# Hawkeye-FineGrained/Hawkeye

Measured on AMD Instinct MI355X. Metric: images/sec (train fwd+bwd) BCNN VGG-16 448^2 bs64, higher is better.
Workload: dtype f32; 1 GPU; BCNN_S2: VGG-16 448x448, per-GPU batch 64, 200 classes, SGD momentum 0.9, CE label_smoothing 0.1, full train step; global_batch=64, parallelism=dp1, memory_format=channels_last

## Files before the change

hawkeye_amd/csrc/api.hip:

```cpp
#include <cstdlib>
#include <cstring>

#include "hk_bgemm.h"
#include "../../include/hawkeye_hip.h"

namespace hk {

namespace {
struct Knob {
    const char* name;
    const char* env;
    int Tuning::*field;
};
const Knob kKnobs[] = {
    {"bcnn_generic", "HK_BCNN_GENERIC", &Tuning::bcnn_generic}, {"cbp_bin", "HK_CBP_BIN", &Tuning::cbp_bin},
    {"roi_bwd", "HK_ROI_BWD", &Tuning::roi_bwd},                {"linear_slabs", "HK_LINEAR_SLABS", &Tuning::linear_slabs},
    {"ns_tn", "HK_NS_TN", &Tuning::ns_tn},                      {"bwd_v", "HK_BWD_V", &Tuning::bwd_v},
    {"ns_streams", "HK_NS_STREAMS", &Tuning::ns_streams},        {"sched_b", "HK_SCHED_B", &Tuning::sched_b},
    {"ns_sym", "HK_NS_SYM", &Tuning::ns_sym},
    {"lin_walk", "HK_LIN_WALK", &Tuning::lin_walk},           {"bwd_fold", "HK_BWD_FOLD", &Tuning::bwd_fold},
    {"fwd_fold", "HK_FWD_FOLD", &Tuning::fwd_fold},             {"conv_wrw", "HK_CONV_WRW", &Tuning::conv_wrw},
    {"wrw_wgs", "HK_WRW_WGS", &Tuning::wrw_wgs},                {"peer_form", "HK_PEER_FORM", &Tuning::peer_form},
    {"wrw_split", "HK_WRW_SPLIT", &Tuning::wrw_split},          {"wrw_wide", "HK_WRW_WIDE", &Tuning::wrw_wide},
    {"conv_fwd", "HK_CONV_FWD", &Tuning::conv_fwd},             {"conv_bwd_data", "HK_CONV_BWD_DATA", &Tuning::conv_bwd_data},
    {"conv_epi", "HK_CONV_EPI", &Tuning::conv_epi},             {"conv_mfma", "HK_CONV_MFMA", &Tuning::conv_mfma},
};
Tuning from_env() {
    Tuning t;
    for (const Knob& k : kKnobs)
        if (const char* e = getenv(k.env)) t.*(k.field) = atoi(e);
    return t;
}
}

Tuning& tuning() {
    static Tuning t = from_env();
    return t;
}

}

using namespace hk;

extern "C" int hk_tuning_set(const char* name, int value) {
    if (!name) return HK_ERR_BAD_ARG;
    for (const Knob& k : kKnobs)
        if (!strcmp(name, k.name)) {
            tuning().*(k.field) = value;
            return HK_OK;
        }
    return HK_ERR_BAD_ARG;
}

extern "C" int hk_tuning_get(const char* name, int* value) {
    if (!name || !value) return HK_ERR_BAD_ARG;
    for (const Knob& k : kKnobs)
        if (!strcmp(name, k.name)) {
            *value = tuning().*(k.field);
            return HK_OK;
        }
    return HK_ERR_BAD_ARG;
}

extern "C" const char* hk_version(void) { return "hawkeye_hip 0.1 gfx950"; }

extern "C" int hk_bgemm_f32(const float* a, int lda, long long stride_a, int trans_a, const float* b, int ldb,
                            long long stride_b, int trans_b, float* c, int ldc, long long stride_c, int M, int N,
                            int K, int batch, float alpha, float beta, float diag, hk_stream_t stream) {
    if (!a || !b || !c) return HK_ERR_BAD_ARG;
    hipStream_t st = (hipStream_t)stream;
    const LdPlain la = trans_a ? make_plain(a, stride_a, lda, K, M) : make_plain(a, stride_a, lda, M, K);
    const LdPlain lb = trans_b ? make_plain(b, stride_b, ldb, N, K) : make_plain(b, stride_b, ldb, K, N);
    const EpAffine ep = make_affine(c, stride_c, ldc, alpha, nullptr, beta, diag);
    if (!trans_a && !trans_b) return bgemm_launch<true, false>(la, lb, ep, M, N, K, batch, st);
    if (!trans_a && trans_b) return bgemm_launch<true, true>(la, lb, ep, M, N, K, batch, st);
    if (trans_a && !trans_b) return bgemm_launch<false, false>(la, lb, ep, M, N, K, batch, st);
    return bgemm_launch<false, true>(la, lb, ep, M, N, K, batch, st);
}
```

hawkeye_amd/csrc/conv_wrw.hip:

```cpp
#include "hk_common.h"
#include "hk_partial_sum.h"
#include "hk_split_bf16.h"
#include "../../include/hawkeye_hip.h"

namespace hk {

constexpr int WRW_CI = 64;
constexpr int WRW_OT = 64;
constexpr int WRW_SW = 32;
constexpr int WRW_XROW = (WRW_SW + 2) * WRW_CI;
constexpr int WRW_DYROW = WRW_SW * WRW_OT;
constexpr int WRW_XF4 = WRW_XROW / 4;
constexpr int WRW_LDS = 4 * WRW_XROW + 2 * WRW_DYROW;
constexpr int WRW_MIN_ROWS = 4;
constexpr int WRW_MAX_WG = 512;

struct WrwStage {
    long long xoff[3], doff[2];
    bool xok[3], dok[2];
};

__device__ __forceinline__ bool wrw_load_x(const float* __restrict__ xi, const WrwStage& st, int r, int H, int W, int cin, f32x4 (&v)[3]) {
    const bool rok = r >= 0 && r < H;
    const float* row = xi + (long long)(r < 0 ? 0 : (r < H ? r : H - 1)) * W * cin;
#pragma unroll
    for (int u = 0; u < 3; ++u) HK_LOAD16_ASYNC(v[u], row + st.xoff[u]);
    return rok;
}
__device__ __forceinline__ void wrw_load_dy(const float* __restrict__ dyi, const WrwStage& st, int h, int H, int W, int Cout, f32x4 (&v)[2]) {
    const float* row = dyi + (long long)(h < H ? h : H - 1) * W * Cout;
#pragma unroll
    for (int u = 0; u < 2; ++u) HK_LOAD16_ASYNC(v[u], row + st.doff[u]);
}
__device__ __forceinline__ void wrw_loads_landed(f32x4 (&vx)[3], f32x4 (&vd)[2]) {
    __builtin_amdgcn_s_waitcnt(HK_VMCNT_IMM(0));
#pragma unroll
    for (int u = 0; u < 3; ++u) HK_PIN_LOADED(vx[u]);
#pragma unroll
    for (int u = 0; u < 2; ++u) HK_PIN_LOADED(vd[u]);
}
__device__ __forceinline__ void wrw_store_x(float* __restrict__ xs, int slot, const WrwStage& st, bool rok, const f32x4 (&v)[3]) {
    const f32x4 zero = {0.f, 0.f, 0.f, 0.f};
    f32x4* d = reinterpret_cast<f32x4*>(xs + slot * WRW_XROW) + threadIdx.x;
    d[0] = (rok && st.xok[0]) ? v[0] : zero;
    d[256] = (rok && st.xok[1]) ? v[1] : zero;
    if (threadIdx.x + 512 < WRW_XF4) d[512] = (rok && st.xok[2]) ? v[2] : zero;
}
__device__ __forceinline__ void wrw_store_dy(float* __restrict__ ds, int buf, const WrwStage& st, const f32x4 (&v)[2]) {
    const f32x4 zero = {0.f, 0.f, 0.f, 0.f};
    f32x4* d = reinterpret_cast<f32x4*>(ds + buf * WRW_DYROW) + threadIdx.x;
    d[0] = st.dok[0] ? v[0] : zero;
    d[256] = st.dok[1] ? v[1] : zero;
}

__global__ __launch_bounds__(256, 2) void conv3x3_wrw_kernel(const float* __restrict__ dy, const float* __restrict__ x,
                                                          float* __restrict__ part, int H, int W, int Cout, int nstrips, int nrb,
                                                          int rpb, int njobs) {
    __shared__ __attribute__((aligned(16))) float lds[WRW_LDS];
    float* xs = lds;
    float* ds = lds + 4 * WRW_XROW;
    const int tid = threadIdx.x, lane = tid & 63, l31 = lane & 31, hf = lane >> 5;
    const int wave = __builtin_amdgcn_readfirstlane(tid >> 6);
    const int oh = wave >> 1, ch = wave & 1;
    const int slice = blockIdx.y;
    const int jb = (int)((long long)blockIdx.x * njobs / gridDim.x), je = (int)((long long)(blockIdx.x + 1) * njobs / gridDim.x);

    f32x16 acc[9];
#pragma unroll
    for (int t = 0; t < 9; ++t)
#pragma unroll
        for (int i = 0; i < 16; ++i) acc[t][i] = 0.f;

    const int aoff = hf * WRW_OT + oh * 32 + l31;
    const int boff = hf * WRW_CI + ch * 32 + l31;

    for (int j = jb; j < je; ++j) {
        const int strip = j % nstrips, jr = j / nstrips;
        const int rb = jr % nrb;
        const long long n = jr / nrb;
        const int c0 = strip * WRW_SW, r0 = rb * rpb;
        const int nrows = (r0 + rpb < H ? r0 + rpb : H) - r0;
        const float* xi = x + n * H * W * WRW_CI;
        const float* dyi = dy + n * H * W * Cout + slice * WRW_OT;
        WrwStage st;
#pragma unroll
        for (int u = 0; u < 3; ++u) {
            const int idx = tid + 256 * u, col = c0 - 1 + (idx >> 4);
            st.xok[u] = idx < WRW_XF4 && col >= 0 && col < W;
            st.xoff[u] = (long long)(col < 0 ? 0 : (col < W ? col : W - 1)) * WRW_CI + 4 * (idx & 15);
        }
#pragma unroll
        for (int u = 0; u < 2; ++u) {
            const int idx = tid + 256 * u, col = c0 + (idx >> 4);
            st.dok[u] = col < W;
            st.doff[u] = (long long)(col < W ? col : W - 1) * Cout + 4 * (idx & 15);
        }
        f32x4 vx[3], vd[2];
        wrw_load_dy(dyi, st, r0, H, W, Cout, vd);
#pragma unroll
        for (int t = 0; t < 3; ++t) {
            const bool rok = wrw_load_x(xi, st, r0 - 1 + t, H, W, WRW_CI, vx);
            wrw_loads_landed(vx, vd);
            wrw_store_x(xs, t, st, rok, vx);
        }
        wrw_store_dy(ds, 0, st, vd);
        __syncthreads();
        for (int k = 0; k < nrows; ++k) {
            const bool rok = wrw_load_x(xi, st, r0 + k + 2, H, W, WRW_CI, vx);
            wrw_load_dy(dyi, st, r0 + k + 1, H, W, Cout, vd);
            const float* A = ds + (k & 1) * WRW_DYROW + aoff;
            const float* B0 = xs + (k & 3) * WRW_XROW + boff;
            const float* B1 = xs + ((k + 1) & 3) * WRW_XROW + boff;
            const float* B2 = xs + ((k + 2) & 3) * WRW_XROW + boff;
            float a = *HK_LDS_CONST(A), b[9];
#pragma unroll
            for (int kw = 0; kw < 3; ++kw) {
                b[kw] = *HK_LDS_CONST(B0 + kw * WRW_CI);
                b[3 + kw] = *HK_LDS_CONST(B1 + kw * WRW_CI);
                b[6 + kw] = *HK_LDS_CONST(B2 + kw * WRW_CI);
            }
#pragma unroll
            for (int p = 0; p < WRW_SW / 2; ++p) {
                float an = 0.f, bn[9];
                if (p + 1 < WRW_SW / 2) {
                    an = *HK_LDS_CONST(A + (2 * p + 2) * WRW_OT);
#pragma unroll
                    for (int kw = 0; kw < 3; ++kw) {
                        bn[kw] = *HK_LDS_CONST(B0 + (2 * p + 2 + kw) * WRW_CI);
                        bn[3 + kw] = *HK_LDS_CONST(B1 + (2 * p + 2 + kw) * WRW_CI);
                        bn[6 + kw] = *HK_LDS_CONST(B2 + (2 * p + 2 + kw) * WRW_CI);
                    }
                }
#pragma unroll
                for (int t = 0; t < 9; ++t) acc[t] = __builtin_amdgcn_mfma_f32_32x32x2f32(a, b[t], acc[t], 0, 0, 0);
                if (p + 1 < WRW_SW / 2) {
                    a = an;
#pragma unroll
                    for (int t = 0; t < 9; ++t) b[t] = bn[t];
                }
            }
            wrw_loads_landed(vx, vd);
            wrw_store_x(xs, (k + 3) & 3, st, rok, vx);
            wrw_store_dy(ds, (k + 1) & 1, st, vd);
            __syncthreads();
        }
    }
    float* pb = part + ((long long)blockIdx.x * Cout + slice * WRW_OT + oh * 32 + 4 * hf) * (9 * WRW_CI) + ch * 32 + l31;
#pragma unroll
    for (int t = 0; t < 9; ++t)
#pragma unroll
        for (int i = 0; i < 16; ++i) pb[(8 * (i >> 2) + (i & 3)) * (9 * WRW_CI) + t * WRW_CI] = acc[t][i];
}

constexpr int WRS_PIX = 32 * 2;
constexpr int WRS_XPLANE = (WRW_SW + 2) * WRS_PIX;
constexpr int WRS_DPLANE = WRW_SW * WRS_PIX;
constexpr int WRS_XSLOT = 6 * WRS_XPLANE;
constexpr int WRS_DBUF = 6 * WRS_DPLANE;
constexpr int WRS_LDS = 4 * WRS_XSLOT + 2 * WRS_DBUF;
constexpr int WRS_FLUSH = 32;

__device__ __forceinline__ void wrs_store(char* base, int plane, f32x4 v) {
    bf16x4 p[3];
    wrs_split(v, p);
#pragma unroll
    for (int s = 0; s < 3; ++s) *reinterpret_cast<bf16x4*>(base + 2 * s * plane) = p[s];
}
__device__ __forceinline__ void wrs_store_x(char* xs, int slot, const WrwStage& st, bool rok, const f32x4 (&v)[3]) {
    const f32x4 zero = {0.f, 0.f, 0.f, 0.f};
    const int tid = threadIdx.x;
    char* d = xs + slot * WRS_XSLOT + ((tid >> 3) & 1) * WRS_XPLANE + (tid >> 4) * WRS_PIX + (tid & 7) * 8;
    wrs_store(d, WRS_XPLANE, (rok && st.xok[0]) ? v[0] : zero);
    wrs_store(d + 16 * WRS_PIX, WRS_XPLANE, (rok && st.xok[1]) ? v[1] : zero);
    if (tid + 512 < WRW_XF4) wrs_store(d + 32 * WRS_PIX, WRS_XPLANE, (rok && st.xok[2]) ? v[2] : zero);
}
__device__ __forceinline__ void wrs_store_dy(char* ds, int buf, const WrwStage& st, const f32x4 (&v)[2]) {
    const f32x4 zero = {0.f, 0.f, 0.f, 0.f};
    const int tid = threadIdx.x;
    char* d = ds + buf * WRS_DBUF + ((tid >> 3) & 1) * WRS_DPLANE + (tid >> 4) * WRS_PIX + (tid & 7) * 8;
    wrs_store(d, WRS_DPLANE, st.dok[0] ? v[0] : zero);
    wrs_store(d + 16 * WRS_PIX, WRS_DPLANE, st.dok[1] ? v[1] : zero);
}
__device__ __forceinline__ bf16x8 wrs_frag(const char* blk, int i) {
#if defined(__HIP_DEVICE_COMPILE__)
    typedef __attribute__((address_space(3))) bf16x4* lds_b64;
    const char* a = blk + (i >> 2) * WRS_PIX + (i & 3) * 8;
    const bf16x4 lo = __builtin_amdgcn_ds_read_tr16_b64_v4bf16((lds_b64)a);
    const bf16x4 hi = __builtin_amdgcn_ds_read_tr16_b64_v4bf16((lds_b64)(a + 4 * WRS_PIX));
    return __builtin_shufflevector(lo, hi, 0, 1, 2, 3, 4, 5, 6, 7);
#else
    bf16x8 f;
    for (int q = 0; q < 8; ++q) {
        __bf16 e;
        __builtin_memcpy(&e, blk + q * WRS_PIX + i * 2, 2);
        f[q] = e;
    }
    return f;
#endif
}

__device__ __forceinline__ void wrs_flush(float* __restrict__ pb, f32x16 (&acc)[9], bool add, int cin) {
#pragma unroll
    for (int t = 0; t < 9; ++t) {
        int o = t * cin;
        HK_PIN_LOADED(o);
        float* q = pb + o;
        f32x16 v = acc[t];
        if (add) {
#pragma unroll
            for (int i = 0; i < 16; ++i) v[i] += q[(8 * (i >> 2) + (i & 3)) * (9 * cin)];
        }
#pragma unroll
        for (int i = 0; i < 16; ++i) {
            q[(8 * (i >> 2) + (i & 3)) * (9 * cin)] = v[i];
            acc[t][i] = 0.f;
        }
        __builtin_amdgcn_sched_barrier(0);
    }
}

template <bool WIDE>
__global__ __launch_bounds__(256, 2) void conv3x3_wrw_split_kernel(const float* __restrict__ dy, const float* __restrict__ x,
                                                                float* __restrict__ part, int H, int W, int Cout, int nstrips,
                                                                int nrb, int rpb, int njobs, int Cin) {
    HK_DYN_LDS16(ldsf);
    char* xs = reinterpret_cast<char*>(ldsf);
    char* ds = xs + 4 * WRS_XSLOT;
    const int tid = threadIdx.x, lane = tid & 63, hf = lane >> 5, l15 = lane & 15;
    const int wave = __builtin_amdgcn_readfirstlane(tid >> 6);
    const int oh = wave >> 1, ch = wave & 1;
    const int cin = WIDE ? Cin : WRW_CI;
    const int slice = blockIdx.y, cslice = WIDE ? blockIdx.z : 0;
    const int jb = (int)((long long)blockIdx.x * njobs / gridDim.x), je = (int)((long long)(blockIdx.x + 1) * njobs / gridDim.x);

    f32x16 acc[9];
#pragma unroll
    for (int t = 0; t < 9; ++t)
#pragma unroll
        for (int i = 0; i < 16; ++i) acc[t][i] = 0.f;

    const int blk = 8 * hf * WRS_PIX + ((lane >> 4) & 1) * 32;
    const int aoff = oh * WRS_DPLANE + blk, boff = ch * WRS_XPLANE + blk;
    auto mine = [&]() {
        const int l = threadIdx.x & 63, w = __builtin_amdgcn_readfirstlane((int)threadIdx.x >> 6);
        return part + ((long long)blockIdx.x * Cout + slice * WRW_OT + (w >> 1) * 32 + 4 * (l >> 5)) * (9 * cin) + cslice * WRW_CI + (w & 1) * 32 + (l & 31);
    };
    int since = 0;
    bool stored = false;

    for (int j = jb; j < je; ++j) {
        const int strip = j % nstrips, jr = j / nstrips;
        const int rb = jr % nrb;
        const long long n = jr / nrb;
        const int c0 = strip * WRW_SW, r0 = rb * rpb;
        const int nrows = (r0 + rpb < H ? r0 + rpb : H) - r0;
        const float* xi = x + n * H * W * cin + cslice * WRW_CI;
        const float* dyi = dy + n * H * W * Cout + slice * WRW_OT;
        WrwStage st;
#pragma unroll
        for (int u = 0; u < 3; ++u) {
            const int idx = tid + 256 * u, col = c0 - 1 + (idx >> 4);
            st.xok[u] = idx < WRW_XF4 && col >= 0 && col < W;
            st.xoff[u] = (long long)(col < 0 ? 0 : (col < W ? col : W - 1)) * cin + 4 * (idx & 15);
        }
#pragma unroll
        for (int u = 0; u < 2; ++u) {
            const int idx = tid + 256 * u, col = c0 + (idx >> 4);
            st.dok[u] = col < W;
            st.doff[u] = (long long)(col < W ? col : W - 1) * Cout + 4 * (idx & 15);
        }
        f32x4 vx[3], vd[2];
        wrw_load_dy(dyi, st, r0, H, W, Cout, vd);
#pragma unroll
        for (int t = 0; t < 3; ++t) {
            const bool rok = wrw_load_x(xi, st, r0 - 1 + t, H, W, cin, vx);
            wrw_loads_landed(vx, vd);
            wrs_store_x(xs, t, st, rok, vx);
        }
        wrs_store_dy(ds, 0, st, vd);
        __syncthreads();
        for (int k = 0; k < nrows; ++k) {
            const bool rok = wrw_load_x(xi, st, r0 + k + 2, H, W, cin, vx);
            wrw_load_dy(dyi, st, r0 + k + 1, H, W, Cout, vd);
            const char* A = ds + (k & 1) * WRS_DBUF + aoff;
            const char* B[3] = {xs + (k & 3) * WRS_XSLOT + boff, xs + ((k + 1) & 3) * WRS_XSLOT + boff, xs + ((k + 2) & 3) * WRS_XSLOT + boff};
            bf16x8 a[3], b[3];
#pragma unroll
            for (int s = 0; s < 3; ++s) {
                a[s] = wrs_frag(A + 2 * s * WRS_DPLANE, l15);
                b[s] = wrs_frag(B[0] + 2 * s * WRS_XPLANE, l15);
            }
#pragma unroll
            for (int i = 0; i < 18; ++i) {
                const int t = i % 9, cn = (i + 1) / 9, tn = (i + 1) % 9;
                bf16x8 an[3], bn[3];
                if (i + 1 < 18) {
#pragma unroll
                    for (int s = 0; s < 3; ++s) {
                        bn[s] = wrs_frag(B[tn / 3] + 2 * s * WRS_XPLANE + (16 * cn + tn % 3) * WRS_PIX, l15);
                        if (tn == 0) an[s] = wrs_frag(A + 2 * s * WRS_DPLANE + 16 * cn * WRS_PIX, l15);
                    }
                }
                __builtin_amdgcn_sched_barrier(0);
                acc[t] = __builtin_amdgcn_mfma_f32_32x32x16_bf16(a[1], b[1], acc[t], 0, 0, 0);
                acc[t] = __builtin_amdgcn_mfma_f32_32x32x16_bf16(a[0], b[2], acc[t], 0, 0, 0);
                acc[t] = __builtin_amdgcn_mfma_f32_32x32x16_bf16(a[2], b[0], acc[t], 0, 0, 0);
                acc[t] = __builtin_amdgcn_mfma_f32_32x32x16_bf16(a[0], b[1], acc[t], 0, 0, 0);
                acc[t] = __builtin_amdgcn_mfma_f32_32x32x16_bf16(a[1], b[0], acc[t], 0, 0, 0);
                acc[t] = __builtin_amdgcn_mfma_f32_32x32x16_bf16(a[0], b[0], acc[t], 0, 0, 0);
                __builtin_amdgcn_sched_barrier(0);
                if (i + 1 < 18) {
#pragma unroll
                    for (int s = 0; s < 3; ++s) {
                        b[s] = bn[s];
                        if (tn == 0) a[s] = an[s];
                    }
                }
            }
            wrw_loads_landed(vx, vd);
            wrs_store_x(xs, (k + 3) & 3, st, rok, vx);
            wrs_store_dy(ds, (k + 1) & 1, st, vd);
            __syncthreads();
            if (++since == WRS_FLUSH) {
                wrs_flush(mine(), acc, stored, cin);
                since = 0;
                stored = true;
            }
        }
    }
    if (since > 0 || !stored) wrs_flush(mine(), acc, stored, cin);
}

static bool wrw_split_wins(int N, int H, int W, int Cout) {
    const long long pixels = (long long)N * H * W;
    return Cout >= 2 * WRW_OT ? pixels >= 16ll * 224 * 224 : pixels >= 32ll * 448 * 448;
}

struct WrwPlan {
    int nstrips, nrb, rpb, njobs, nwg;
};
static int wrw_wide_wgs(long long slices) { return slices < 512 ? (int)(512 / slices) : 1; }

static bool wrw_plan(int N, int H, int W, int slices, bool wide, WrwPlan& pl) {
    const int room = wide ? wrw_wide_wgs(slices) : WRW_MAX_WG;
    int wgmax = tuning().wrw_wgs > 0 ? tuning().wrw_wgs : (wide ? room : (slices <= 8 ? 512 / slices : 64));
    if (wgmax > room) wgmax = room;
    const long long nstrips = ((long long)W + WRW_SW - 1) / WRW_SW, base = (long long)N * nstrips;
    long long best = -1;
    for (int cand = 1; cand <= (H / WRW_MIN_ROWS > 1 ? H / WRW_MIN_ROWS : 1); ++cand) {
        const int rpb = (H + cand - 1) / cand, nrb = (H + rpb - 1) / rpb;
        if (nrb != cand) continue;
        const long long jobs = base * nrb;
        if (jobs > 0x7fffffffll) break;
        const long long wg = jobs < wgmax ? jobs : wgmax;
        const long long cost = ((jobs + wg - 1) / wg) * (rpb + 2);
        if (best < 0 || cost < best) {
            best = cost;
            pl.nstrips = (int)nstrips; pl.nrb = nrb; pl.rpb = rpb; pl.njobs = (int)jobs; pl.nwg = (int)wg;
        }
    }
    return best >= 0;
}

}

using namespace hk;

extern "C" size_t hk_conv3x3_wrw_ws_bytes(int Cin, int Cout) {
    if (Cin <= 0 || Cout <= 0) return 0;
    const size_t one = (size_t)Cout * 9 * Cin * sizeof(float);
    if (Cin <= WRW_CI) return WRW_MAX_WG * one;
    return wrw_wide_wgs(((long long)Cin + WRW_CI - 1) / WRW_CI * (((long long)Cout + WRW_OT - 1) / WRW_OT)) * one;
}

extern "C" int hk_conv3x3_wrw(const float* dy, const float* x, float* dw, int N, int H, int W, int Cin, int Cout, void* ws,
                              size_t ws_bytes, hk_stream_t stream) {
    if (!dy || !x || !dw || N <= 0 || H <= 0 || W <= 0 || Cin <= 0 || Cout <= 0) return HK_ERR_BAD_ARG;
    if (!ws || ws_bytes < hk_conv3x3_wrw_ws_bytes(Cin, Cout)) return HK_ERR_WORKSPACE;
    if (Cin % WRW_CI != 0 || Cout % WRW_OT != 0 || Cout / WRW_OT > 65535 || Cin / WRW_CI > 65535 || (long long)Cout * 9 * Cin > 0x7fffffffll ||
        !aligned16(dy) || !aligned16(x) || !aligned16(dw) || !aligned16(ws))
        return HK_ERR_UNSUPPORTED;
    const int split = tuning().wrw_split;
    const bool wide = Cin > WRW_CI;
    if (wide && (split == 0 || tuning().wrw_wide == 0)) return HK_ERR_UNSUPPORTED;
    const int oslices = Cout / WRW_OT, cslices = Cin / WRW_CI;
    if ((long long)oslices * cslices > 0x7fffffffll) return HK_ERR_UNSUPPORTED;
    WrwPlan pl;
    if (!wrw_plan(N, H, W, oslices * cslices, wide, pl)) return HK_ERR_UNSUPPORTED;
    float* part = (float*)ws;
    if (wide) {
        HK_ALLOW_BIG_LDS(conv3x3_wrw_split_kernel<true>, WRS_LDS);
        hipLaunchKernelGGL(conv3x3_wrw_split_kernel<true>, dim3((unsigned)pl.nwg, (unsigned)oslices, (unsigned)cslices), dim3(256), WRS_LDS,
                           (hipStream_t)stream, dy, x, part, H, W, Cout, pl.nstrips, pl.nrb, pl.rpb, pl.njobs, Cin);
    } else if (split > 0 || (split < 0 && wrw_split_wins(N, H, W, Cout))) {
        HK_ALLOW_BIG_LDS(conv3x3_wrw_split_kernel<false>, WRS_LDS);
        hipLaunchKernelGGL(conv3x3_wrw_split_kernel<false>, dim3((unsigned)pl.nwg, (unsigned)(Cout / WRW_OT)), dim3(256), WRS_LDS,
                           (hipStream_t)stream, dy, x, part, H, W, Cout, pl.nstrips, pl.nrb, pl.rpb, pl.njobs, WRW_CI);
    } else {
        hipLaunchKernelGGL(conv3x3_wrw_kernel, dim3((unsigned)pl.nwg, (unsigned)(Cout / WRW_OT)), dim3(256), 0, (hipStream_t)stream, dy, x,
                           part, H, W, Cout, pl.nstrips, pl.nrb, pl.rpb, pl.njobs);
    }
    HK_LAUNCH_CHECK();
    const int nel = Cout * 9 * Cin;
    hipLaunchKernelGGL(partial_sum_kernel<16>, dim3((nel + 63) / 64), dim3(1024), 0, (hipStream_t)stream, (const float*)part, pl.nwg, nel, nel,
                       dw, (float*)nullptr);
    HK_LAUNCH_CHECK();
    return HK_OK;
}
```

hawkeye_amd/csrc/hk_common.h:

```cpp
#pragma once
#include <hip/hip_runtime.h>
#include <stdint.h>
#include <stddef.h>
#include <mutex>

typedef float f32x2 __attribute__((ext_vector_type(2)));
typedef float f32x4 __attribute__((ext_vector_type(4)));
typedef float f32x16 __attribute__((ext_vector_type(16)));

#define HK_OK 0
#define HK_ERR_BAD_ARG (-1)
#define HK_ERR_WORKSPACE (-2)
#define HK_ERR_UNSUPPORTED (-3)

#include <hk_isa.h>

#define HK_VMCNT_IMM(n) (((n) & 15) | (((n) >> 4) << 14) | (7 << 4) | (15 << 8))
#define HK_VM_BARRIER(n)                                                                                       \
    do {                                                                                                       \
        asm volatile("" ::: "memory");                                         \
        __builtin_amdgcn_s_waitcnt(HK_VMCNT_IMM(n));                                                           \
        __builtin_amdgcn_s_barrier();                                                                          \
        asm volatile("" ::: "memory");                                                                         \
    } while (0)

#define HK_LAUNCH_CHECK()                                 \
    do {                                                  \
        hipError_t e__ = hipGetLastError();               \
        if (e__ != hipSuccess) return (int)e__;           \
    } while (0)

namespace hk {

struct Tuning {
    int bcnn_generic = 0;
    int cbp_bin = -1;
    int roi_bwd = 0;
    int linear_slabs = 0;
    int ns_tn = 0;
    int bwd_v = 0;
    int ns_streams = 1;
    int ns_sym = 1;
    int lin_walk = -1;
    int fwd_fold = 0;
    int bwd_fold = 0;
    int sched_b = 0;
    int conv_wrw = 1;
    int wrw_wgs = 0;
    int wrw_split = -1;
    int wrw_wide = 1;
    int conv_fwd = -1;
    int conv_bwd_data = -1;
    int conv_epi = 2;
    int conv_mfma = -1;
    int peer_form = 0;
};
Tuning& tuning();

constexpr int HK_MAX_AUX = 3;
struct AuxQueue {
    hipStream_t aux[HK_MAX_AUX] = {nullptr, nullptr, nullptr};
    hipEvent_t fork = nullptr, join[HK_MAX_AUX] = {nullptr, nullptr, nullptr};
    bool ok = false;
    std::mutex busy;
};
inline AuxQueue* aux_queue(hipStream_t st) {
    static AuxQueue tab[16];
    static std::once_flag once[16];
    int dev = 0, sdev = 0;
    if (hipGetDevice(&dev) != hipSuccess || dev < 0 || dev >= 16) return nullptr;
    if (st != nullptr && (hipStreamGetDevice(st, &sdev) != hipSuccess || sdev != dev)) return nullptr;
    AuxQueue& a = tab[dev];
    std::call_once(once[dev], [&a]() {
        bool good = hipEventCreateWithFlags(&a.fork, hipEventDisableTiming) == hipSuccess;
        for (int i = 0; i < HK_MAX_AUX && good; ++i)
            good = hipStreamCreateWithFlags(&a.aux[i], hipStreamNonBlocking) == hipSuccess &&
                   hipEventCreateWithFlags(&a.join[i], hipEventDisableTiming) == hipSuccess;
        if (!good) {
            for (int i = 0; i < HK_MAX_AUX; ++i) {
                if (a.join[i]) (void)hipEventDestroy(a.join[i]);
                if (a.aux[i]) (void)hipStreamDestroy(a.aux[i]);
                a.join[i] = nullptr; a.aux[i] = nullptr;
            }
            if (a.fork) (void)hipEventDestroy(a.fork);
            a.fork = nullptr;
        }
        a.ok = good;
    });
    return a.ok ? &a : nullptr;
}
class AuxScope {
  public:
    AuxScope(hipStream_t st, int n) : st_(st) {
        if (n <= 0) return;
        if (n > HK_MAX_AUX) n = HK_MAX_AUX;
        q_ = aux_queue(st);
        if (!q_) return;
        q_->busy.lock();
        bool good = hipEventRecord(q_->fork, st_) == hipSuccess;
        for (int i = 0; i < n && good; ++i) good = hipStreamWaitEvent(q_->aux[i], q_->fork, 0) == hipSuccess;
        if (good) {
            n_ = n;
        } else {
            q_->busy.unlock();
            q_ = nullptr;
        }
    }
    AuxScope(const AuxScope&) = delete;
    AuxScope& operator=(const AuxScope&) = delete;
    ~AuxScope() { (void)join(); }
    int count() const { return n_; }
    hipStream_t aux(int i) const { return q_->aux[i]; }
    int join() {
        if (!n_) return HK_OK;
        hipError_t e = hipSuccess;
        for (int i = 0; i < n_; ++i) {
            hipError_t r = hipEventRecord(q_->join[i], q_->aux[i]);
            if (r == hipSuccess) r = hipStreamWaitEvent(st_, q_->join[i], 0);
            if (e == hipSuccess) e = r;
        }
        n_ = 0;
        q_->busy.unlock();
        q_ = nullptr;
        return e == hipSuccess ? HK_OK : (int)e;
    }

  private:
    hipStream_t st_;
    int n_ = 0;
    AuxQueue* q_ = nullptr;
};

constexpr int WAVE = 64;
constexpr int NXCD = 8;

template <int AUX = 0>
__device__ __forceinline__ void glds16(const float* g, float* l) {
    __builtin_amdgcn_global_load_lds((const __attribute__((address_space(1))) void*)g,
                                     (__attribute__((address_space(3))) void*)l, 16, 0, AUX);
}

__device__ __forceinline__ void glds4(const float* g, float* l) {
    __builtin_amdgcn_global_load_lds((const __attribute__((address_space(1))) void*)g,
                                     (__attribute__((address_space(3))) void*)l, 4, 0, 0);
}

__device__ __forceinline__ float wave_sum(float v) {
#pragma unroll
    for (int o = 32; o > 0; o >>= 1) v += __shfl_xor(v, o, 64);
    return v;
}

__device__ __forceinline__ float wave_max(float v) {
#pragma unroll
    for (int o = 32; o > 0; o >>= 1) v = fmaxf(v, __shfl_xor(v, o, 64));
    return v;
}

template <int NW>
__device__ __forceinline__ float block_sum(float v, float* red) {
    v = wave_sum(v);
    const int w = threadIdx.x >> 6;
    __syncthreads();
    if ((threadIdx.x & 63) == 0) red[w] = v;
    __syncthreads();
    float s = 0.f;
#pragma unroll
    for (int i = 0; i < NW; ++i) s += red[i];
    return s;
}

__host__ __device__ __forceinline__ int xcd_grid(int nb, int tiles) {
    return (nb >= NXCD) ? NXCD * ((nb + NXCD - 1) / NXCD) * tiles : nb * tiles;
}
__device__ __forceinline__ bool xcd_map(int bid, int nb, int tiles, int& sample, int& tile) {
    if (nb >= NXCD) {
        const int xcd = bid % NXCD, slot = bid / NXCD;
        sample = xcd + NXCD * (slot / tiles);
        tile = slot % tiles;
    } else {
        sample = bid / tiles;
        tile = bid % tiles;
    }
    return sample < nb;
}

__host__ __forceinline__ bool aligned16(const void* p) { return (((uintptr_t)p) & 15) == 0; }

#define HK_ALLOW_BIG_LDS(fn, bytes)                                                                            \
    do {                                                                                                       \
        static size_t have_[32] = {0};                                                                         \
        int dev_ = 0;                                                                                          \
        if (hipGetDevice(&dev_) != hipSuccess || dev_ < 0 || dev_ > 31) dev_ = 0;                             \
        if ((size_t)(bytes) > 64 * 1024 && (size_t)(bytes) > have_[dev_]) {                                    \
            const hipError_t e_ = hipFuncSetAttribute(reinterpret_cast<const void*>(fn),                      \
                                                      hipFuncAttributeMaxDynamicSharedMemorySize, (int)(bytes)); \
            if (e_ != hipSuccess) return (int)e_;                                                              \
            have_[dev_] = (size_t)(bytes);                                                                     \
        }                                                                                                      \
    } while (0)

}
```

Before: 592.9 images/sec.

## Add 16x16x32 bf16 MFMA variant of split-bf16 conv weight-gradient kernel

Adds a second instantiation of the split-precision 3x3 conv weight-gradient kernel that uses 16x16x32 bf16 MFMAs instead of 32x32x16. It has its own LDS layout, with a padded pitch and a permuted K pixel order, and static_asserts that check bank-conflict-free transposing reads and staging stores. The variant is selected by default through a new wrw_mfma knob whose heuristic always picks it. The aim is better MFMA throughput and conflict-free LDS access, at the cost of more fragment reads per MFMA and a different accumulator layout in the flush.

```diff
diff --git a/hawkeye_amd/csrc/api.hip b/hawkeye_amd/csrc/api.hip
--- a/hawkeye_amd/csrc/api.hip
+++ b/hawkeye_amd/csrc/api.hip
@@ -24,6 +24,7 @@
     {"wrw_split", "HK_WRW_SPLIT", &Tuning::wrw_split},          {"wrw_wide", "HK_WRW_WIDE", &Tuning::wrw_wide},
     {"conv_fwd", "HK_CONV_FWD", &Tuning::conv_fwd},             {"conv_bwd_data", "HK_CONV_BWD_DATA", &Tuning::conv_bwd_data},
     {"conv_epi", "HK_CONV_EPI", &Tuning::conv_epi},             {"conv_mfma", "HK_CONV_MFMA", &Tuning::conv_mfma},
+    {"wrw_mfma", "HK_WRW_MFMA", &Tuning::wrw_mfma},
 };
 Tuning from_env() {
     Tuning t;
diff --git a/hawkeye_amd/csrc/conv_wrw.hip b/hawkeye_amd/csrc/conv_wrw.hip
--- a/hawkeye_amd/csrc/conv_wrw.hip
+++ b/hawkeye_amd/csrc/conv_wrw.hip
@@ -1,6 +1,7 @@
 #include "hk_common.h"
 #include "hk_partial_sum.h"
 #include "hk_split_bf16.h"
+#include <hk_mfma_bf16.h>
 #include "../../include/hawkeye_hip.h"
 
 namespace hk {
@@ -160,26 +161,26 @@
 constexpr int WRS_LDS = 4 * WRS_XSLOT + 2 * WRS_DBUF;
 constexpr int WRS_FLUSH = 32;
 
-__device__ __forceinline__ void wrs_store(char* base, int plane, f32x4 v) {
+__device__ __forceinline__ void wrs_store(char* base, int piece, f32x4 v) {
     bf16x4 p[3];
     wrs_split(v, p);
 #pragma unroll
-    for (int s = 0; s < 3; ++s) *reinterpret_cast<bf16x4*>(base + 2 * s * plane) = p[s];
+    for (int s = 0; s < 3; ++s) *reinterpret_cast<bf16x4*>(base + s * piece) = p[s];
 }
 __device__ __forceinline__ void wrs_store_x(char* xs, int slot, const WrwStage& st, bool rok, const f32x4 (&v)[3]) {
     const f32x4 zero = {0.f, 0.f, 0.f, 0.f};
     const int tid = threadIdx.x;
     char* d = xs + slot * WRS_XSLOT + ((tid >> 3) & 1) * WRS_XPLANE + (tid >> 4) * WRS_PIX + (tid & 7) * 8;
-    wrs_store(d, WRS_XPLANE, (rok && st.xok[0]) ? v[0] : zero);
-    wrs_store(d + 16 * WRS_PIX, WRS_XPLANE, (rok && st.xok[1]) ? v[1] : zero);
-    if (tid + 512 < WRW_XF4) wrs_store(d + 32 * WRS_PIX, WRS_XPLANE, (rok && st.xok[2]) ? v[2] : zero);
+    wrs_store(d, 2 * WRS_XPLANE, (rok && st.xok[0]) ? v[0] : zero);
+    wrs_store(d + 16 * WRS_PIX, 2 * WRS_XPLANE, (rok && st.xok[1]) ? v[1] : zero);
+    if (tid + 512 < WRW_XF4) wrs_store(d + 32 * WRS_PIX, 2 * WRS_XPLANE, (rok && st.xok[2]) ? v[2] : zero);
 }
 __device__ __forceinline__ void wrs_store_dy(char* ds, int buf, const WrwStage& st, const f32x4 (&v)[2]) {
     const f32x4 zero = {0.f, 0.f, 0.f, 0.f};
     const int tid = threadIdx.x;
     char* d = ds + buf * WRS_DBUF + ((tid >> 3) & 1) * WRS_DPLANE + (tid >> 4) * WRS_PIX + (tid & 7) * 8;
-    wrs_store(d, WRS_DPLANE, st.dok[0] ? v[0] : zero);
-    wrs_store(d + 16 * WRS_PIX, WRS_DPLANE, st.dok[1] ? v[1] : zero);
+    wrs_store(d, 2 * WRS_DPLANE, st.dok[0] ? v[0] : zero);
+    wrs_store(d + 16 * WRS_PIX, 2 * WRS_DPLANE, st.dok[1] ? v[1] : zero);
 }
 __device__ __forceinline__ bf16x8 wrs_frag(const char* blk, int i) {
 #if defined(__HIP_DEVICE_COMPILE__)
@@ -219,13 +220,134 @@
     }
 }
 
-template <bool WIDE>
+constexpr int WRS_MF_32 = 0, WRS_MF_16 = 1;
+constexpr int WRS16_PIX = 16 * 2;
+constexpr int WRS16_PITCH = WRW_SW + 3;
+constexpr int WRS16_QPLANE = WRS16_PITCH * WRS16_PIX;
+constexpr int WRS16_PIECE = 4 * WRS16_QPLANE;
+constexpr int WRS16_SLOT = 3 * WRS16_PIECE;
+constexpr int WRS16_LDS = 6 * WRS16_SLOT;
+
+__host__ __device__ constexpr int wrs16_off(int piece, int quarter, int pixel, int ch) {
+    return piece * WRS16_PIECE + quarter * WRS16_QPLANE + pixel * WRS16_PIX + ch * 2;
+}
+__host__ __device__ constexpr int wrs16_kpix(int g, int e) { return 16 * (e >> 2) + 4 * g + (e & 3); }
+constexpr bool wrs16_reads_conflict_free() {
+    for (int piece = 0; piece < 3; ++piece)
+        for (int quarter = 0; quarter < 4; ++quarter)
+            for (int kw = 0; kw < 3; ++kw)
+                for (int rd = 0; rd < 2; ++rd)
+                    for (int half = 0; half < 2; ++half) {
+                        unsigned long long seen = 0;
+                        for (int l = 32 * half; l < 32 * half + 32; ++l) {
+                            const int g = l >> 4, i = l & 15;
+                            const int a = wrs16_off(piece, quarter, kw + wrs16_kpix(g, 4 * rd) + (i >> 2), 4 * (i & 3));
+                            if (a % 8 != 0 || kw + wrs16_kpix(g, 4 * rd + 3) >= WRS16_PITCH) return false;
+                            for (int d = 0; d < 2; ++d) {
+                                const int bank = (a / 4 + d) % 64;
+                                if ((seen >> bank) & 1ull) return false;
+                                seen |= 1ull << bank;
+                            }
+                        }
+                    }
+    return true;
+}
+constexpr bool wrs16_stores_conflict_free() {
+    for (int u = 0; u < 3; ++u)
+        for (int grp = 0; grp < 16; ++grp) {
+            unsigned seen = 0;
+            for (int tid = 16 * grp; tid < 16 * grp + 16; ++tid) {
+                const int a = wrs16_off(0, (tid >> 2) & 3, (tid >> 4) + 16 * u, 4 * (tid & 3));
+                for (int d = 0; d < 2; ++d) {
+                    const int bank = (a / 4 + d) % 32;
+                    if ((seen >> bank) & 1u) return false;
+                    seen |= 1u << bank;
+                }
+            }
+        }
+    return true;
+}
+constexpr bool wrs16_k_is_a_permutation() {
+    unsigned seen = 0;
+    for (int g = 0; g < 4; ++g)
+        for (int e = 0; e < 8; ++e) seen |= 1u << wrs16_kpix(g, e);
+    return seen == 0xffffffffu;
+}
+static_assert(wrs16_reads_conflict_free(), "both 32-lane halves of both transposing reads of a WRS_MF_16 fragment cover the 64 banks once, at every kw");
+static_assert(wrs16_stores_conflict_free(), "every 16-lane group of a WRS_MF_16 staging store covers the 32 banks once");
+static_assert(wrs16_k_is_a_permutation(), "the four groups' fragments hold the strip row's 32 pixels once each");
+static_assert(2 * WRS16_LDS <= 160 * 1024 && WRS16_PITCH >= WRW_SW + 2, "two workgroups per CU; a plane holds an x row segment");
+
+__device__ __forceinline__ void wrs16_store_x(char* xs, int slot, const WrwStage& st, bool rok, const f32x4 (&v)[3]) {
+    const f32x4 zero = {0.f, 0.f, 0.f, 0.f};
+    const int tid = threadIdx.x;
+    char* d = xs + slot * WRS16_SLOT + wrs16_off(0, (tid >> 2) & 3, tid >> 4, 4 * (tid & 3));
+    wrs_store(d, WRS16_PIECE, (rok && st.xok[0]) ? v[0] : zero);
+    wrs_store(d + 16 * WRS16_PIX, WRS16_PIECE, (rok && st.xok[1]) ? v[1] : zero);
+    if (tid + 512 < WRW_XF4) wrs_store(d + 32 * WRS16_PIX, WRS16_PIECE, (rok && st.xok[2]) ? v[2] : zero);
+}
+__device__ __forceinline__ void wrs16_store_dy(char* ds, int buf, const WrwStage& st, const f32x4 (&v)[2]) {
+    const f32x4 zero = {0.f, 0.f, 0.f, 0.f};
+    const int tid = threadIdx.x;
+    char* d = ds + buf * WRS16_SLOT + wrs16_off(0, (tid >> 2) & 3, tid >> 4, 4 * (tid & 3));
+    wrs_store(d, WRS16_PIECE, st.dok[0] ? v[0] : zero);
+    wrs_store(d + 16 * WRS16_PIX, WRS16_PIECE, st.dok[1] ? v[1] : zero);
+}
+__device__ __forceinline__ bf16x8 wrs16_frag(const char* blk, int g, int i) {
+#if defined(__HIP_DEVICE_COMPILE__)
+    typedef __attribute__((address_space(3))) bf16x4* lds_b64;
+    const char* a = blk + wrs16_off(0, 0, wrs16_kpix(g, 0) + (i >> 2), 4 * (i & 3));
+    const bf16x4 lo = __builtin_amdgcn_ds_read_tr16_b64_v4bf16((lds_b64)a);
+    const bf16x4 hi = __builtin_amdgcn_ds_read_tr16_b64_v4bf16((lds_b64)(a + (wrs16_kpix(0, 4) - wrs16_kpix(0, 0)) * WRS16_PIX));
+    return __builtin_shufflevector(lo, hi, 0, 1, 2, 3, 4, 5, 6, 7);
+#else
+    bf16x8 f;
+    for (int e = 0; e < 8; ++e) {
+        __bf16 v;
+        __builtin_memcpy(&v, blk + wrs16_off(0, 0, wrs16_kpix(g, e), i), 2);
+        f[e] = v;
+    }
+    return f;
+#endif
+}
+__device__ __forceinline__ void wrs16_flush(float* __restrict__ pb, f32x4 (&acc)[9][2][2], bool add, int cin) {
+#pragma unroll
+    for (int t = 0; t < 9; ++t) {
+        int o = t * cin;
+        HK_PIN_LOADED(o);
+        float* q = pb + o;
+        f32x4 v[2][2];
+#pragma unroll
+        for (int ob = 0; ob < 2; ++ob)
+#pragma unroll
+            for (int cb = 0; cb < 2; ++cb) {
+                v[ob][cb] = acc[t][ob][cb];
+                if (add) {
+#pragma unroll
+                    for (int e = 0; e < 4; ++e) v[ob][cb][e] += q[(16 * ob + e) * (9 * cin) + 16 * cb];
+                }
+            }
+#pragma unroll
+        for (int ob = 0; ob < 2; ++ob)
+#pragma unroll
+            for (int cb = 0; cb < 2; ++cb)
+#pragma unroll
+                for (int e = 0; e < 4; ++e) {
+                    q[(16 * ob + e) * (9 * cin) + 16 * cb] = v[ob][cb][e];
+                    acc[t][ob][cb][e] = 0.f;
+                }
+        __builtin_amdgcn_sched_barrier(0);
+    }
+}
+
+template <bool WIDE, int MF>
 __global__ __launch_bounds__(256, 2) void conv3x3_wrw_split_kernel(const float* __restrict__ dy, const float* __restrict__ x,
                                                                 float* __restrict__ part, int H, int W, int Cout, int nstrips,
                                                                 int nrb, int rpb, int njobs, int Cin) {
+    constexpr bool M32 = MF == WRS_MF_32;
     HK_DYN_LDS16(ldsf);
     char* xs = reinterpret_cast<char*>(ldsf);
-    char* ds = xs + 4 * WRS_XSLOT;
+    char* ds = xs + 4 * (M32 ? WRS_XSLOT : WRS16_SLOT);
     const int tid = threadIdx.x, lane = tid & 63, hf = lane >> 5, l15 = lane & 15;
     const int wave = __builtin_amdgcn_readfirstlane(tid >> 6);
     const int oh = wave >> 1, ch = wave & 1;
@@ -234,16 +356,27 @@
     const int jb = (int)((long long)blockIdx.x * njobs / gridDim.x), je = (int)((long long)(blockIdx.x + 1) * njobs / gridDim.x);
 
     f32x16 acc[9];
-#pragma unroll
-    for (int t = 0; t < 9; ++t)
-#pragma unroll
-        for (int i = 0; i < 16; ++i) acc[t][i] = 0.f;
+    f32x4 acc4[9][2][2];
+    if constexpr (M32) {
+#pragma unroll
+        for (int t = 0; t < 9; ++t)
+#pragma unroll
+            for (int i = 0; i < 16; ++i) acc[t][i] = 0.f;
+    } else {
+#pragma unroll
+        for (int t = 0; t < 9; ++t)
+#pragma unroll
+            for (int q = 0; q < 4; ++q) acc4[t][q >> 1][q & 1] = (f32x4){0.f, 0.f, 0.f, 0.f};
+    }
 
     const int blk = 8 * hf * WRS_PIX + ((lane >> 4) & 1) * 32;
-    const int aoff = oh * WRS_DPLANE + blk, boff = ch * WRS_XPLANE + blk;
+    const int aoff = M32 ? oh * WRS_DPLANE + blk : wrs16_off(0, 2 * oh, 0, 0), boff = M32 ? ch * WRS_XPLANE + blk : wrs16_off(0, 2 * ch, 0, 0);
     auto mine = [&]() {
         const int l = threadIdx.x & 63, w = __builtin_amdgcn_readfirstlane((int)threadIdx.x >> 6);
-        return part + ((long long)blockIdx.x * Cout + slice * WRW_OT + (w >> 1) * 32 + 4 * (l >> 5)) * (9 * cin) + cslice * WRW_CI + (w & 1) * 32 + (l & 31);
+        if constexpr (M32)
+            return part + ((long long)blockIdx.x * Cout + slice * WRW_OT + (w >> 1) * 32 + 4 * (l >> 5)) * (9 * cin) + cslice * WRW_CI + (w & 1) * 32 + (l & 31);
+        else
+            return part + ((long long)blockIdx.x * Cout + slice * WRW_OT + (w >> 1) * 32 + 4 * (l >> 4)) * (9 * cin) + cslice * WRW_CI + (w & 1) * 32 + (l & 15);
     };
     int since = 0;
     bool stored = false;
@@ -275,65 +408,113 @@
         for (int t = 0; t < 3; ++t) {
             const bool rok = wrw_load_x(xi, st, r0 - 1 + t, H, W, cin, vx);
             wrw_loads_landed(vx, vd);
-            wrs_store_x(xs, t, st, rok, vx);
-        }
-        wrs_store_dy(ds, 0, st, vd);
+            if constexpr (M32) wrs_store_x(xs, t, st, rok, vx);
+            else wrs16_store_x(xs, t, st, rok, vx);
+        }
+        if constexpr (M32) wrs_store_dy(ds, 0, st, vd);
+        else wrs16_store_dy(ds, 0, st, vd);
         __syncthreads();
         for (int k = 0; k < nrows; ++k) {
             const bool rok = wrw_load_x(xi, st, r0 + k + 2, H, W, cin, vx);
             wrw_load_dy(dyi, st, r0 + k + 1, H, W, Cout, vd);
-            const char* A = ds + (k & 1) * WRS_DBUF + aoff;
-            const char* B[3] = {xs + (k & 3) * WRS_XSLOT + boff, xs + ((k + 1) & 3) * WRS_XSLOT + boff, xs + ((k + 2) & 3) * WRS_XSLOT + boff};
-            bf16x8 a[3], b[3];
-#pragma unroll
-            for (int s = 0; s < 3; ++s) {
-                a[s] = wrs_frag(A + 2 * s * WRS_DPLANE, l15);
-                b[s] = wrs_frag(B[0] + 2 * s * WRS_XPLANE, l15);
-            }
-#pragma unroll
-            for (int i = 0; i < 18; ++i) {
-                const int t = i % 9, cn = (i + 1) / 9, tn = (i + 1) % 9;
-                bf16x8 an[3], bn[3];
-                if (i + 1 < 18) {
-#pragma unroll
-                    for (int s = 0; s < 3; ++s) {
-                        bn[s] = wrs_frag(B[tn / 3] + 2 * s * WRS_XPLANE + (16 * cn + tn % 3) * WRS_PIX, l15);
-                        if (tn == 0) an[s] = wrs_frag(A + 2 * s * WRS_DPLANE + 16 * cn * WRS_PIX, l15);
+            constexpr int DBUF = M32 ? WRS_DBUF : WRS16_SLOT, XSLOT = M32 ? WRS_XSLOT : WRS16_SLOT;
+            const char* A = ds + (k & 1) * DBUF + aoff;
+            const char* B[3] = {xs + (k & 3) * XSLOT + boff, xs + ((k + 1) & 3) * XSLOT + boff, xs + ((k + 2) & 3) * XSLOT + boff};
+            if constexpr (!M32) {
+                const int g = lane >> 4;
+                constexpr int PA[6] = {1, 0, 2, 0, 1, 0}, PB[6] = {1, 2, 0, 1, 0, 0};
+                bf16x8 a[2][3], b[3];
+#pragma unroll
+                for (int pr = 0; pr < 3; ++pr) {
+#pragma unroll
+                    for (int ob = 0; ob < 2; ++ob) a[ob][PA[pr]] = wrs16_frag(A + wrs16_off(PA[pr], ob, 0, 0), g, l15);
+                    b[PB[pr]] = wrs16_frag(B[0] + wrs16_off(PB[pr], 0, 0, 0), g, l15);
+                }
+#pragma unroll
+                for (int i = 0; i < 18; ++i) {
+                    const int t = i / 2, cb = i % 2, tn = (i + 1) / 2, cbn = (i + 1) % 2;
+                    bf16x8 bn[3];
+                    if (i + 1 < 18) {
+#pragma unroll
+                        for (int s = 0; s < 3; ++s) bn[s] = wrs16_frag(B[tn / 3] + wrs16_off(s, cbn, tn % 3, 0), g, l15);
                     }
-                }
-                __builtin_amdgcn_sched_barrier(0);
-                acc[t] = __builtin_amdgcn_mfma_f32_32x32x16_bf16(a[1], b[1], acc[t], 0, 0, 0);
-                acc[t] = __builtin_amdgcn_mfma_f32_32x32x16_bf16(a[0], b[2], acc[t], 0, 0, 0);
-                acc[t] = __builtin_amdgcn_mfma_f32_32x32x16_bf16(a[2], b[0], acc[t], 0, 0, 0);
-                acc[t] = __builtin_amdgcn_mfma_f32_32x32x16_bf16(a[0], b[1], acc[t], 0, 0, 0);
-                acc[t] = __builtin_amdgcn_mfma_f32_32x32x16_bf16(a[1], b[0], acc[t], 0, 0, 0);
-                acc[t] = __builtin_amdgcn_mfma_f32_32x32x16_bf16(a[0], b[0], acc[t], 0, 0, 0);
-                __builtin_amdgcn_sched_barrier(0);
-                if (i + 1 < 18) {
-#pragma unroll
-                    for (int s = 0; s < 3; ++s) {
-                        b[s] = bn[s];
-                        if (tn == 0) a[s] = an[s];
+                    __builtin_amdgcn_sched_barrier(0);
+#pragma unroll
+                    for (int pr = 0; pr < 6; ++pr)
+#pragma unroll
+                        for (int ob = 0; ob < 2; ++ob) acc4[t][ob][cb] = mfma_f32_16x16x32_bf16(a[ob][PA[pr]], b[PB[pr]], acc4[t][ob][cb]);
+                    __builtin_amdgcn_sched_barrier(0);
+                    if (i + 1 < 18) {
+#pragma unroll
+                        for (int s = 0; s < 3; ++s) b[s] = bn[s];
+                    }
+                }
+            } else {
+                bf16x8 a[3], b[3];
+#pragma unroll
+                for (int s = 0; s < 3; ++s) {
+                    a[s] = wrs_frag(A + 2 * s * WRS_DPLANE, l15);
+                    b[s] = wrs_frag(B[0] + 2 * s * WRS_XPLANE, l15);
+                }
+#pragma unroll
+                for (int i = 0; i < 18; ++i) {
+                    const int t = i % 9, cn = (i + 1) / 9, tn = (i + 1) % 9;
+                    bf16x8 an[3], bn[3];
+                    if (i + 1 < 18) {
+#pragma unroll
+                        for (int s = 0; s < 3; ++s) {
+                            bn[s] = wrs_frag(B[tn / 3] + 2 * s * WRS_XPLANE + (16 * cn + tn % 3) * WRS_PIX, l15);
+                            if (tn == 0) an[s] = wrs_frag(A + 2 * s * WRS_DPLANE + 16 * cn * WRS_PIX, l15);
+                        }
+                    }
+                    __builtin_amdgcn_sched_barrier(0);
+                    acc[t] = __builtin_amdgcn_mfma_f32_32x32x16_bf16(a[1], b[1], acc[t], 0, 0, 0);
+                    acc[t] = __builtin_amdgcn_mfma_f32_32x32x16_bf16(a[0], b[2], acc[t], 0, 0, 0);
+                    acc[t] = __builtin_amdgcn_mfma_f32_32x32x16_bf16(a[2], b[0], acc[t], 0, 0, 0);
+                    acc[t] = __builtin_amdgcn_mfma_f32_32x32x16_bf16(a[0], b[1], acc[t], 0, 0, 0);
+                    acc[t] = __builtin_amdgcn_mfma_f32_32x32x16_bf16(a[1], b[0], acc[t], 0, 0, 0);
+                    acc[t] = __builtin_amdgcn_mfma_f32_32x32x16_bf16(a[0], b[0], acc[t], 0, 0, 0);
+                    __builtin_amdgcn_sched_barrier(0);
+                    if (i + 1 < 18) {
+#pragma unroll
+                        for (int s = 0; s < 3; ++s) {
+                            b[s] = bn[s];
+                            if (tn == 0) a[s] = an[s];
+                        }
                     }
                 }
             }
             wrw_loads_landed(vx, vd);
-            wrs_store_x(xs, (k + 3) & 3, st, rok, vx);
-            wrs_store_dy(ds, (k + 1) & 1, st, vd);
+            if constexpr (M32) {
+                wrs_store_x(xs, (k + 3) & 3, st, rok, vx);
+                wrs_store_dy(ds, (k + 1) & 1, st, vd);
+            } else {
+                wrs16_store_x(xs, (k + 3) & 3, st, rok, vx);
+                wrs16_store_dy(ds, (k + 1) & 1, st, vd);
+            }
             __syncthreads();
             if (++since == WRS_FLUSH) {
-                wrs_flush(mine(), acc, stored, cin);
+                if constexpr (M32) wrs_flush(mine(), acc, stored, cin);
+                else wrs16_flush(mine(), acc4, stored, cin);
                 since = 0;
                 stored = true;
             }
         }
     }
-    if (since > 0 || !stored) wrs_flush(mine(), acc, stored, cin);
+    if (since > 0 || !stored) {
+        if constexpr (M32) wrs_flush(mine(), acc, stored, cin);
+        else wrs16_flush(mine(), acc4, stored, cin);
+    }
 }
 
 static bool wrw_split_wins(int N, int H, int W, int Cout) {
     const long long pixels = (long long)N * H * W;
     return Cout >= 2 * WRW_OT ? pixels >= 16ll * 224 * 224 : pixels >= 32ll * 448 * 448;
+}
+
+static bool wrw_mfma16_wins(int N, int H, int W, int Cout) {
+    (void)N; (void)H; (void)W; (void)Cout;
+    return true;
 }
 
 struct WrwPlan {
@@ -362,6 +543,17 @@
     return best >= 0;
 }
 
+template <bool WIDE, int MF>
+static int wrw_split_launch(dim3 grid, const float* dy, const float* x, float* part, int H, int W, int Cout, const WrwPlan& pl, int cin,
+                            hk_stream_t stream) {
+    constexpr int LDS = MF == WRS_MF_32 ? WRS_LDS : WRS16_LDS;
+    HK_ALLOW_BIG_LDS((conv3x3_wrw_split_kernel<WIDE, MF>), LDS);
+    hipLaunchKernelGGL((conv3x3_wrw_split_kernel<WIDE, MF>), grid, dim3(256), LDS, (hipStream_t)stream, dy, x, part, H, W, Cout, pl.nstrips,
+                       pl.nrb, pl.rpb, pl.njobs, cin);
+    HK_LAUNCH_CHECK();
+    return HK_OK;
+}
+
 }
 
 using namespace hk;
@@ -388,14 +580,18 @@
     WrwPlan pl;
     if (!wrw_plan(N, H, W, oslices * cslices, wide, pl)) return HK_ERR_UNSUPPORTED;
     float* part = (float*)ws;
+    const int mfma = tuning().wrw_mfma;
+    const bool mf16 = mfma == 1 || (mfma < 0 && wrw_mfma16_wins(N, H, W, Cout));
     if (wide) {
-        HK_ALLOW_BIG_LDS(conv3x3_wrw_split_kernel<true>, WRS_LDS);
-        hipLaunchKernelGGL(conv3x3_wrw_split_kernel<true>, dim3((unsigned)pl.nwg, (unsigned)oslices, (unsigned)cslices), dim3(256), WRS_LDS,
-                           (hipStream_t)stream, dy, x, part, H, W, Cout, pl.nstrips, pl.nrb, pl.rpb, pl.njobs, Cin);
+        const dim3 grid((unsigned)pl.nwg, (unsigned)oslices, (unsigned)cslices);
+        const int e = mf16 ? wrw_split_launch<true, WRS_MF_16>(grid, dy, x, part, H, W, Cout, pl, Cin, stream)
+                           : wrw_split_launch<true, WRS_MF_32>(grid, dy, x, part, H, W, Cout, pl, Cin, stream);
+        if (e != HK_OK) return e;
     } else if (split > 0 || (split < 0 && wrw_split_wins(N, H, W, Cout))) {
-        HK_ALLOW_BIG_LDS(conv3x3_wrw_split_kernel<false>, WRS_LDS);
-        hipLaunchKernelGGL(conv3x3_wrw_split_kernel<false>, dim3((unsigned)pl.nwg, (unsigned)(Cout / WRW_OT)), dim3(256), WRS_LDS,
-                           (hipStream_t)stream, dy, x, part, H, W, Cout, pl.nstrips, pl.nrb, pl.rpb, pl.njobs, WRW_CI);
+        const dim3 grid((unsigned)pl.nwg, (unsigned)(Cout / WRW_OT));
+        const int e = mf16 ? wrw_split_launch<false, WRS_MF_16>(grid, dy, x, part, H, W, Cout, pl, WRW_CI, stream)
+                           : wrw_split_launch<false, WRS_MF_32>(grid, dy, x, part, H, W, Cout, pl, WRW_CI, stream);
+        if (e != HK_OK) return e;
     } else {
         hipLaunchKernelGGL(conv3x3_wrw_kernel, dim3((unsigned)pl.nwg, (unsigned)(Cout / WRW_OT)), dim3(256), 0, (hipStream_t)stream, dy, x,
                            part, H, W, Cout, pl.nstrips, pl.nrb, pl.rpb, pl.njobs);
diff --git a/hawkeye_amd/csrc/hk_common.h b/hawkeye_amd/csrc/hk_common.h
--- a/hawkeye_amd/csrc/hk_common.h
+++ b/hawkeye_amd/csrc/hk_common.h
@@ -49,6 +49,7 @@
     int wrw_wgs = 0;
     int wrw_split = -1;
     int wrw_wide = 1;
+    int wrw_mfma = -1;
     int conv_fwd = -1;
     int conv_bwd_data = -1;
     int conv_epi = 2;
```

Result: faster. 601.6 images/sec, median of 6 (+1.5%).
